# zyang1580/PDA

Measured on AMD Instinct MI355X. Metric: users/sec full-catalogue top-K@50 (eval), higher is better.
Workload: dtype f32; 1 GPU; C3: synthetic 1000000 users x 200000 items, d=128, PDA condition ((elu+1)*pop^0.22) head, masked top-K@50; ranks_seen=1

## Files before the change

pda_amd/csrc/pda_score_topk_v4.hip:

```cpp
#include "pda_v4_shared.h"
#include <cstdlib>
#include <type_traits>

using namespace pda_topk;

namespace {

constexpr int kCap4 = 57;
constexpr int kRing4 = 128;
constexpr int kWarmTiles = 4;
constexpr int kMainWaves = 8;
#ifndef PDA_W4_ABL
#define PDA_W4_ABL 0
#endif
#ifdef PDA_V4_PROF
__device__ unsigned long long pda_prof4[24];
#define PROF_T0(v) const long long v = __builtin_readcyclecounter()
#define PROF_T1(v, slot) prof[slot] += (unsigned long long)(__builtin_readcyclecounter() - v)
#define PROF_INC(slot, x) prof[slot] += (unsigned long long)(x)
#define PROF_FLUSH(first, last) do { if (lane == 0) for (int pq = (first); pq <= (last); ++pq) atomicAdd(&pda_prof4[pq], prof[pq]); } while (0)
#else
#define PROF_T0(v) do {} while (0)
#define PROF_T1(v, slot) do {} while (0)
#define PROF_INC(slot, x) do {} while (0)
// ... 565 lines not shown
        const int row = (r & 3) + 8 * (r >> 2) + 4 * h;
        const int lrow = wave * 32 + row;
        if (j == 0) predt[lrow] = c_t >= K ? pda_unordf(t) : -INFINITY;
        if (__any(c_t > cap_t)) {
#pragma unroll
            for (int k = 0; k < NHT; ++k) {
                const bool p = ordv[k][r] >= t;
                const uint64_t key = ((uint64_t)ordv[k][r] << 32) | (uint64_t)(0xFFFFFFFFu - (uint32_t)itemv[k]);
                append_keys<CAP>(p, lrow, pda_unordf(ordv[k][r]), key, lists, cntl, taul, wave * 32, 32, K, lane);
            }
        } else {
            int run = 0;
#pragma unroll
            for (int k = 0; k < NHT; ++k) {
                const bool p = ordv[k][r] >= t;
                const uint64_t bm = __ballot(p);
                const uint32_t bh = h ? (uint32_t)(bm >> 32) : (uint32_t)bm;
                const int slot = run + __popc(bh & ((1u << j) - 1u));
                if (p) lists[(size_t)lrow * CAP + slot] = ((uint64_t)ordv[k][r] << 32) | (uint64_t)(0xFFFFFFFFu - (uint32_t)itemv[k]);
                run += __popc(bh);
            }
            if (j == 0) cntl[lrow] = run;
        }
    };
#pragma unroll
    for (int r = 0; r < 16; r += 2) {
        if constexpr ((PDA_W4_ABL & 2) != 0) {
#if defined(__HIP_DEVICE_COMPILE__)
#pragma unroll
            for (int k = 0; k < NHT; ++k) asm volatile("" ::"v"(ordv[k][r]), "v"(ordv[k][r + 1]));
#endif
            continue;
        }
        auto count_ge2 = [&](uint32_t ca, uint32_t cb, int& na, int& nb) __attribute__((always_inline)) {
            int loa = 0, hia = 0, lob = 0, hib = 0;
#pragma unroll
            for (int k = 0; k < NHT; ++k) {
                const uint64_t bma = __ballot(ordv[k][r] >= ca);
                const uint64_t bmb = __ballot(ordv[k][r + 1] >= cb);
                loa += __popc((uint32_t)bma);
                hia += __popc((uint32_t)(bma >> 32));
                lob += __popc((uint32_t)bmb);
                hib += __popc((uint32_t)(bmb >> 32));
            }
            na = h ? hia : loa;
            nb = h ? hib : lob;
        };
        int ca_t, cb_t;
        count_ge2(1u, 1u, ca_t, cb_t);
        uint32_t ta = 1u, tb = 1u;
        const bool needa = ca_t > cap_t, needb = cb_t > cap_t;
        if (__any(needa || needb)) {
            uint32_t mxa = 0u, mna = 0xFFFFFFFFu, mxb = 0u, mnb = 0xFFFFFFFFu;
#pragma unroll
            for (int k = 0; k < NHT; ++k) {
                const uint32_t va = ordv[k][r], vb = ordv[k][r + 1];
                mxa = max(mxa, va);
                mna = min(mna, va != 0u ? va : 0xFFFFFFFFu);
                mxb = max(mxb, vb);
                mnb = min(mnb, vb != 0u ? vb : 0xFFFFFFFFu);
            }
#pragma unroll
            for (int o = 16; o >= 1; o >>= 1) {
                mxa = max(mxa, (uint32_t)__shfl_xor((int)mxa, o, 64));
                mna = min(mna, (uint32_t)__shfl_xor((int)mna, o, 64));
                mxb = max(mxb, (uint32_t)__shfl_xor((int)mxb, o, 64));
                mnb = min(mnb, (uint32_t)__shfl_xor((int)mnb, o, 64));
            }
            uint32_t hia = mxa + 1u, hib = mxb + 1u;
            if (needa) ta = mna;
            if (needb) tb = mnb;
            for (int it = 0; it < 40; ++it) {
                const bool opena = needa && ca_t > cap_t && hia - ta > 1u;
                const bool openb = needb && cb_t > cap_t && hib - tb > 1u;
                if (!__any(opena || openb)) break;
                const uint32_t mida = opena ? ta + ((hia - ta) >> 1) : ta;
                const uint32_t midb = openb ? tb + ((hib - tb) >> 1) : tb;
                int cnta, cntb;
                count_ge2(mida, midb, cnta, cntb);
                if (opena) {
                    if (cnta >= K) {
                        ta = mida;
                        ca_t = cnta;
                    } else {
                        hia = mida;
                    }
                }
                if (openb) {
                    if (cntb >= K) {
                        tb = midb;
                        cb_t = cntb;
                    } else {
                        hib = midb;
                    }
                }
            }
        }
        emit_row(r, ta, ca_t);
        emit_row(r + 1, tb, cb_t);
    }
    pda_wave_sync();
    if (tid == 0) atomicAdd(reinterpret_cast<unsigned long long*>(g.stats + 2), (unsigned long long)(2 * nwarm));
    for (int rr = 0; rr < 32; ++rr) {
        uint64_t* buf = my_lists + rr * CAP;
        if (((PDA_W4_ABL & 4) == 0) && (g.warm_sorted || g.warm_final || (g.handover == nullptr && __builtin_amdgcn_readfirstlane(cntl[wave * 32 + rr]) > K)))
            compact_list<CAP>(buf, &cntl[wave * 32 + rr], &taul[wave * 32 + rr], K, lane);
        const int c = cntl[wave * 32 + rr];
        const int rb = utile * kUserTile + wave * 32 + rr;
        if (g.seed_out != nullptr) {
            uint32_t mn = lane < c ? (uint32_t)(buf[lane] >> 32) : 0xFFFFFFFFu;
#pragma unroll
            for (int o = 32; o >= 1; o >>= 1) mn = min(mn, (uint32_t)__shfl_xor((int)mn, o, 64));
            if (lane == 0 && rb < g.n_users_blk) g.seed_out[rb] = c >= K ? pda_unordf(mn) : -INFINITY;
        }
        if (g.kth_ws != nullptr) continue;
        if (g.handover != nullptr) {
            if (rb < g.n_users_blk && lane < CAP) g.handover[((size_t)split * g.n_users_blk + rb) * CAP + lane] = lane < c ? buf[lane] : 0ull;
            if (g.warm_final && rb < g.n_users_blk && lane < K) g.out_keys[((size_t)split * g.n_users_blk + rb) * K + lane] = lane < c ? buf[lane] : 0ull;
        } else if (rb < g.n_users_blk && lane < K) {
            const uint64_t k = lane < c ? buf[lane] : 0ull;
            g.out_keys[((size_t)split * g.n_users_blk + rb) * K + lane] = k;
        }
    }
    if (g.kth_ws != nullptr) {
        pda_wave_sync();
        const int rb0 = utile * kUserTile + wave * 32, nv = max(0, min(32, g.n_users_blk - rb0));
        if (lane < nv) {
            const uint64_t kl = my_lists[(size_t)lane * CAP + (K - 1)];
            g.kth_ws[(size_t)split * g.n_users_blk + rb0 + lane] = cntl[wave * 32 + lane] >= K ? pda_unordf((uint32_t)(kl >> 32)) : -INFINITY;
        }
        uint64_t* ob = g.out_keys + ((size_t)split * g.n_users_blk + rb0) * K;
        const int q64 = 64 / K, r64 = 64 % K;
        int rr = lane / K, p = lane % K;
        for (int i = lane; i < nv * K; i += 64) {
            ob[i] = p < cntl[wave * 32 + rr] ? my_lists[(size_t)rr * CAP + p] : 0ull;
            rr += q64;
            p += r64;
            if (p >= K) { p -= K; ++rr; }
        }
    }
    if (g.pred_ws != nullptr && lane < 32) {
        const int rb = utile * kUserTile + wave * 32 + lane;
        if (rb < g.n_users_blk) {
            g.pred_ws[2 * (size_t)rb] = predt[wave * 32 + lane];
            g.pred_ws[2 * (size_t)rb + 1] = nul[wave * 32 + lane];
        }
    }
}

constexpr int kWS5Waves = 8, kWS5Threads = 64 * kWS5Waves;
constexpr int kWarmPos = 64 * kWarmTiles;
constexpr size_t warm_score5_lds(int d) { return (size_t)kWarmPos * d * 4 + kWarmPos * 8 + (size_t)kWS5Waves * 32 * 2 * kWarmTiles * 4; }

template <int D, bool BF>
__global__ void __launch_bounds__(kWS5Threads) warm_score5_kernel(Args4 g) {
    extern __shared__ __attribute__((aligned(16))) unsigned char smem[];
    constexpr int RB = row_bytes(D);
    constexpr int NC = D / 8;
    constexpr int CPR4 = D / 4;
    float* Bt = reinterpret_cast<float*>(smem);
    float* popw = Bt + kWarmPos * D;
    int* idw = reinterpret_cast<int*>(popw + kWarmPos);
    unsigned* hmask = reinterpret_cast<unsigned*>(idw + kWarmPos);

    const int tid = threadIdx.x, lane = tid & 63, wave = tid >> 6;
    const int j = lane & 31, h = lane >> 5;
    const int nwarm = g.warm_tiles;
    const int npos = 64 * nwarm;
    for (int p = tid; p < npos; p += kWS5Threads) {
        const float* tl = reinterpret_cast<const float*>(g.rows + (size_t)p * RB + 2 * D + 32);
        popw[p] = tl[0];
        idw[p] = reinterpret_cast<const int*>(tl)[1];
    }
    __syncthreads();
    for (int id = tid; id < npos * CPR4; id += kWS5Threads) {
        const int jj = id / CPR4, ch = id % CPR4;
        *reinterpret_cast<f32x4*>(Bt + jj * D + 4 * (ch ^ swz<D>(jj & 31))) = pda_load4<BF>(g.I, (size_t)idw[jj] * D + 4 * ch);
    }
    if (blockIdx.x == 0) {
        for (int p = tid; p < kWarmPos; p += kWS5Threads) g.wscore[p] = p < npos ? (uint32_t)idw[p] : 0u;
        if (tid == 0) g.stats[8] = 5u;
    }
    __syncthreads();

    uint32_t* scores = g.wscore + kWarmPos;
    const int utiles_w = (g.n_users_blk + kUserTile - 1) / kUserTile;
    const int nunits = utiles_w * (kUserTile / 32);
    const int G = (int)gridDim.x, stride = G * kWS5Waves;
    unsigned* hm_l = hmask + wave * 32 * 2 * kWarmTiles;
    static_assert(2 * kWarmTiles == 8, "two 16-byte loads per row");

    auto row_uid = [&](int unit) -> int {
        const int rb = unit * 32 + j;
        return (unit < nunits && rb < g.n_users_blk) ? g.users[rb] : 0;
    };
    auto load_rows = [&](int unit_x, int uid, f32x4 (&a)[NC], u32x4& hm, bool& hm_on) __attribute__((always_inline)) {
        if (unit_x >= nunits) return;
        const int rb = unit_x * 32 + j;
#pragma unroll
        for (int c = 0; c < NC; ++c) a[c] = pda_load4<BF>(g.U, (size_t)uid * D + 4 * h + 8 * c);
        hm_on = false;
        if (g.hmask_tab != nullptr) {
            hm_on = rb < g.n_users_blk && (unsigned)uid < (unsigned)g.hmask_tab_rows;
            hm = *reinterpret_cast<const u32x4*>(g.hmask_tab + (size_t)(hm_on ? uid : 0) * (2 * kWarmTiles) + 4 * h);
        } else if (g.hmask_ws != nullptr) {
            hm_on = true;
            hm = *reinterpret_cast<const u32x4*>(g.hmask_ws + (size_t)rb * (2 * kWarmTiles) + 4 * h);
        }
    };
    unsigned long long n_tiles_done = 0ull;
    auto run_unit = [&](const int unit_in, f32x4 (&areg)[NC], const u32x4& hm_in, const bool hm_on) __attribute__((always_inline)) {
        const int unit = __builtin_amdgcn_readfirstlane(unit_in);
        const int row_blk = unit * 32 + j;
        if (unit * 32 + 32 > g.n_users_blk) {
            const f32x4 z = {0.f, 0.f, 0.f, 0.f};
#pragma unroll
            for (int c = 0; c < NC; ++c) areg[c] = row_blk < g.n_users_blk ? areg[c] : z;
        }
        const u32x4 hz = {0u, 0u, 0u, 0u};
        const u32x4 hmv = hm_on ? hm_in : hz;
        *reinterpret_cast<u32x4*>(hm_l + j * (2 * kWarmTiles) + 4 * h) = hmv;
        {
            constexpr int NK5 = D / 32;
            unsigned char* fb = g.ufrag_out + ((size_t)(row_blk >> 4) * (NK5 * 64) + (size_t)(row_blk & 15)) * 16 + 8 * h;
            float ssc[NC];
#pragma unroll
            for (int c = 0; c < NC; ++c) {
                const f32x4 v = areg[c];
                uint2 w;
                w.x = bf16_rne(v[0]) | (bf16_rne(v[1]) << 16);
                w.y = bf16_rne(v[2]) | (bf16_rne(v[3]) << 16);
                *reinterpret_cast<uint2*>(fb + ((c >> 2) * 64 + 16 * (c & 3)) * 16) = w;
                float ss = 0.f;
#pragma unroll
                for (int k = 0; k < 4; ++k) {
                    const float sq = v[k] * v[k];
                    ss += sq + __shfl_xor(sq, 32, 64);
                }
                ssc[c] = ss;
                __builtin_amdgcn_sched_barrier(0);
            }
#pragma unroll
            for (int o = NC / 2; o > 0; o >>= 1)
#pragma unroll
                for (int c = 0; c < o; ++c) ssc[c] += ssc[c + o];
            if (h == 0) g.unorm_out[row_blk] = sqrtf(ssc[0]) * 1.0009765625f * 1.0001f;
        }
        if ((unit & (kUserTile / 32 - 1)) == 0) n_tiles_done += (unsigned long long)(2 * nwarm);
        pda_wave_sync();
        const int j_lane = j, h_lane = h;
#pragma unroll 1
        for (int ht = 0; ht < 2 * nwarm; ++ht) {
            int j = j_lane, h = h_lane;
#if defined(__HIP_DEVICE_COMPILE__)
            asm volatile("" : "+v"(j), "+v"(h));
#endif
            const int bswz = swz<D>(j);
            const float* brow = Bt + (ht * 32 + j) * D;
            f32x16 acc0 = zero16v(), acc1 = zero16v();
            f32x4 b0 = *reinterpret_cast<const f32x4*>(brow + 4 * (h ^ bswz));
            f32x4 b1 = *reinterpret_cast<const f32x4*>(brow + 4 * ((2 + h) ^ bswz));
#pragma unroll
            for (int c = 0; c < NC; c += 2) {
                f32x4 n0 = b0, n1 = b1;
                if (c + 2 < NC) {
                    n0 = *reinterpret_cast<const f32x4*>(brow + 4 * ((2 * c + 4 + h) ^ bswz));
                    n1 = *reinterpret_cast<const f32x4*>(brow + 4 * ((2 * c + 6 + h) ^ bswz));
                }
#pragma unroll
                for (int q = 0; q < 4; ++q) {
                    acc0 = __builtin_amdgcn_mfma_f32_32x32x2f32(areg[c][q], b0[q], acc0, 0, 0, 0);
                    acc1 = __builtin_amdgcn_mfma_f32_32x32x2f32(areg[c + 1][q], b1[q], acc1, 0, 0, 0);
                }
                __builtin_amdgcn_sched_barrier(0);
                b0 = n0;
                b1 = n1;
            }
            const f32x16 accx = acc0 + acc1;
            const bool okw = (ht * 32 + j) < g.n_items_local;
            const float pv = popw[ht * 32 + j];
            const unsigned hb_mine = hm_l[j * (2 * kWarmTiles) + ht];
            const bool any_hb = __any(hb_mine != 0u);
            const uint32_t soff = (uint32_t)(unit * 32 + 4 * h) * (uint32_t)npos + (uint32_t)(ht * 32 + j);
#pragma unroll
            for (int r = 0; r < 16; ++r) {
                const int row = (r & 3) + 8 * (r >> 2) + 4 * h;
                float sc = accx[r];
                sc = (sc > 0.0f ? sc + 1.0f : __expf(sc)) * pv;
                bool p = okw && (sc >= -INFINITY);
                if (any_hb) {
                    const uint32_t hbr = (uint32_t)__shfl((int)hb_mine, row, 64);
                    if ((hbr >> j) & 1u) p = false;
                }
                scores[soff + (uint32_t)((r & 3) + 8 * (r >> 2)) * (uint32_t)npos] = p ? pda_ordf(sc + 0.0f) : 0u;
            }
        }
        pda_wave_sync();
    };
    int unit = (int)blockIdx.x + G * wave;
    f32x4 ra[NC], rb_[NC];
    u32x4 ha = {0u, 0u, 0u, 0u}, hb = {0u, 0u, 0u, 0u};
    bool oa = false, ob = false;
    load_rows(unit, row_uid(unit), ra, ha, oa);
    int uid_n = row_uid(unit + stride);
    while (unit < nunits) {
        load_rows(unit + stride, uid_n, rb_, hb, ob);
        uid_n = row_uid(unit + 2 * stride);
        run_unit(unit, ra, ha, oa);
        unit += stride;
        if (unit >= nunits) break;
        load_rows(unit + stride, uid_n, ra, ha, oa);
        uid_n = row_uid(unit + 2 * stride);
        run_unit(unit, rb_, hb, ob);
        unit += stride;
    }
    if (lane == 0 && n_tiles_done != 0ull) atomicAdd(reinterpret_cast<unsigned long long*>(g.stats + 2), n_tiles_done);
    if ((int)blockIdx.x == (nunits - 1) % G) {
        const size_t r0 = (size_t)utiles_w * kUserTile, r1 = ((size_t)g.n_users_blk + kUT5 - 1) / kUT5 * kUT5;
        const u32x4 z = {0u, 0u, 0u, 0u};
        for (size_t q = r0 * (2 * D) + (size_t)tid * 16; q < r1 * (2 * D); q += (size_t)kWS5Threads * 16) *reinterpret_cast<u32x4*>(g.ufrag_out + q) = z;
        for (size_t r = r0 + tid; r < r1; r += kWS5Threads) g.unorm_out[r] = 0.f;
    }
}

constexpr int kSelRows = 16;
__global__ void __launch_bounds__(256) __attribute__((amdgpu_waves_per_eu(8))) warm_select5_kernel(Args4 g) {
    constexpr int CAP = kCap4;
    __shared__ uint64_t lists[4][2][64];
    const int tid = threadIdx.x, lane = tid & 63, wave = tid >> 6;
    const int K = g.K, n = g.n_users_blk;
    const int npos = 64 * g.warm_tiles;
    const uint32_t* scores = g.wscore + kWarmPos;
    const int rb0 = ((int)blockIdx.x * 4 + wave) * kSelRows;
    if (rb0 >= n) return;
    const u32x4 idv = *reinterpret_cast<const u32x4*>(g.wscore + 4 * lane);
    uint32_t klo[4];
#pragma unroll
    for (int q = 0; q < 4; ++q) klo[q] = 0xFFFFFFFFu - (uint32_t)(g.item_offset + (int)idv[q]);
    const bool lane_on = 4 * lane < npos;
    float kth_mine = -INFINITY;

    auto count32 = [&](const u32x4& v, uint32_t t) __attribute__((always_inline)) -> int {
        return __popcll(__ballot(v[0] >= t)) + __popcll(__ballot(v[1] >= t)) + __popcll(__ballot(v[2] >= t)) + __popcll(__ballot(v[3] >= t));
    };
    auto key_of = [&](const u32x4& v, int q) __attribute__((always_inline)) -> uint64_t { return ((uint64_t)v[q] << 32) | (uint64_t)klo[q]; };
    auto count64 = [&](const u32x4& v, uint64_t t) __attribute__((always_inline)) -> int {
        int c = 0;
#pragma unroll
        for (int q = 0; q < 4; ++q) c += __popcll(__ballot(key_of(v, q) >= t));
        return c;
    };

#pragma unroll 1
    for (int it = 0; it < kSelRows; it += 2) {
        if (rb0 + it >= n) break;
        u32x4 v[2];
        uint32_t t[2], hi[2];
        int ct[2];
        bool need[2];
#pragma unroll
        for (int s = 0; s < 2; ++s) {
            const int rb = rb0 + it + s;
            const u32x4 z = {0u, 0u, 0u, 0u};
            v[s] = (lane_on && rb < n) ? *reinterpret_cast<const u32x4*>(scores + (size_t)rb * npos + 4 * lane) : z;
        }
#pragma unroll
        for (int s = 0; s < 2; ++s) {
            ct[s] = count32(v[s], 1u);
            t[s] = 1u;
            hi[s] = 0u;
            need[s] = ct[s] > CAP;
        }
        if (need[0] || need[1]) {
#pragma unroll
            for (int s = 0; s < 2; ++s) {
                uint32_t mx = max(max(v[s][0], v[s][1]), max(v[s][2], v[s][3])), mn = 0xFFFFFFFFu;
#pragma unroll
                for (int q = 0; q < 4; ++q) mn = min(mn, v[s][q] != 0u ? v[s][q] : 0xFFFFFFFFu);
#pragma unroll
                for (int o = 32; o >= 1; o >>= 1) {
                    mx = max(mx, (uint32_t)__shfl_xor((int)mx, o, 64));
                    mn = min(mn, (uint32_t)__shfl_xor((int)mn, o, 64));
                }
                hi[s] = (uint32_t)__builtin_amdgcn_readfirstlane((int)mx) + 1u;
                if (need[s]) t[s] = (uint32_t)__builtin_amdgcn_readfirstlane((int)mn);
            }
            for (int step = 0; step < 40; ++step) {
                const bool open0 = need[0] && ct[0] > CAP && hi[0] - t[0] > 1u;
                const bool open1 = need[1] && ct[1] > CAP && hi[1] - t[1] > 1u;
                if (!(open0 || open1)) break;
                const uint32_t mid0 = open0 ? t[0] + ((hi[0] - t[0]) >> 1) : t[0];
                const uint32_t mid1 = open1 ? t[1] + ((hi[1] - t[1]) >> 1) : t[1];
                const int c0 = count32(v[0], mid0), c1 = count32(v[1], mid1);
                if (open0) {
                    if (c0 >= K) { t[0] = mid0; ct[0] = c0; } else { hi[0] = mid0; }
                }
                if (open1) {
                    if (c1 >= K) { t[1] = mid1; ct[1] = c1; } else { hi[1] = mid1; }
                }
            }
        }
        uint64_t thr[2];
#pragma unroll
        for (int s = 0; s < 2; ++s) {
            thr[s] = (uint64_t)t[s] << 32;
            if (ct[s] > CAP) {
                uint64_t lo64 = thr[s], hi64 = (uint64_t)(t[s] + 1u) << 32;
                for (int step = 0; step < 40 && ct[s] > CAP && hi64 - lo64 > 1ull; ++step) {
                    const uint64_t mid = lo64 + ((hi64 - lo64) >> 1);
                    const int c = count64(v[s], mid);
                    if (c >= K) { lo64 = mid; ct[s] = c; } else { hi64 = mid; }
                }
                thr[s] = lo64;
            }
        }
        int cs[2];
#pragma unroll
        for (int s = 0; s < 2; ++s) {
            uint64_t* buf = lists[wave][s];
            int run = 0;
#pragma unroll
            for (int q = 0; q < 4; ++q) {
                const uint64_t key = key_of(v[s], q);
                const bool p = key >= thr[s];
                const uint64_t bm = __ballot(p);
                const int slot = run + (int)__builtin_amdgcn_mbcnt_hi((uint32_t)(bm >> 32), __builtin_amdgcn_mbcnt_lo((uint32_t)bm, 0));
                if (p && slot < 64) buf[slot] = key;
                run += __popcll(bm);
            }
            cs[s] = min(run, CAP);
            if (lane >= cs[s]) buf[lane] = 0ull;
        }
        pda_wave_sync();
        uint64_t key[2];
        int rank[2] = {0, 0};
        key[0] = lists[wave][0][lane];
        key[1] = lists[wave][1][lane];
        const int cm = max(cs[0], cs[1]);
        for (int jj = 0; jj < cm; jj += 4) {
#pragma unroll
            for (int s = 0; s < 2; ++s) {
                const uint64_t* buf = lists[wave][s];
                const uint64_t k0 = buf[jj], k1 = buf[jj + 1], k2 = buf[jj + 2], k3 = buf[jj + 3];
                rank[s] += ((k0 > key[s]) ? 1 : 0) + ((k1 > key[s]) ? 1 : 0) + ((k2 > key[s]) ? 1 : 0) + ((k3 > key[s]) ? 1 : 0);
            }
        }
        pda_wave_sync();
#pragma unroll
        for (int s = 0; s < 2; ++s)
            if (lane < cs[s]) lists[wave][s][rank[s]] = key[s];
        pda_wave_sync();
#pragma unroll
        for (int s = 0; s < 2; ++s) {
            const int rb = rb0 + it + s;
            if (rb < n) {
                if (lane < K) g.out_keys[(size_t)rb * K + lane] = lists[wave][s][lane];
                const uint64_t kl = lists[wave][s][K - 1];
                if (lane == it + s) kth_mine = cs[s] >= K ? pda_unordf((uint32_t)(kl >> 32)) : -INFINITY;
            }
        }
        pda_wave_sync();
    }
    if (lane < kSelRows && rb0 + lane < n) {
        g.kth_ws[rb0 + lane] = kth_mine;
        if (g.seed_out != nullptr) g.seed_out[rb0 + lane] = kth_mine;
    }
}


// ... 1172 lines not shown
    if (mask_from_table) {
        g.hmask_tab = mask_table;
        g.hmask_tab_rows = mask_table_rows;
    }
    if (c.mask_kernel) g.hmask_ws = reinterpret_cast<uint32_t*>(wsb + W.hmask);
    if (c.regroup) {
        g.regroup_ws = reinterpret_cast<int32_t*>(wsb + W.regroup);
        if (phase & 1) g.pred_ws = reinterpret_cast<float*>(g.regroup_ws + 1024 + 2 * (size_t)n_users_blk);
    }

    if (counters_reset && hipMemsetAsync(workspace, 0, W.lists, s) != hipSuccess) return PDA_ERR_LAUNCH;
    if (c.bloom) {
        hipLaunchKernelGGL(hist_bloom4_kernel, dim3((unsigned)((n_users_blk + 31) / 32)), dim3(256), 0, s, users, hist_indptr, hist_indices,
                           hist_row_mode, n_users_blk, const_cast<uint32_t*>(g.bloom), g.prep_hdr, pop_head ? 1 : 0);
        PDA_CHECK_LAUNCH();
    }
#define PDA_V4_(DD, BFV) (pop_head ? launch4<DD, PDA_HEAD_POP, BFV>(g, c, s) : launch4<DD, PDA_HEAD_RAW, BFV>(g, c, s))
    switch (d) {
        case 64: return bf16 ? PDA_V4_(64, true) : PDA_V4_(64, false);
        case 128: return bf16 ? PDA_V4_(128, true) : PDA_V4_(128, false);
        case 256: return bf16 ? PDA_V4_(256, true) : PDA_V4_(256, false);
        default: return PDA_ERR_UNSUPPORTED;
    }
#undef PDA_V4_
}

__global__ void __launch_bounds__(256) kth_value_kernel(const uint64_t* __restrict__ keys, int S, int n_users, int K, int pos, float* __restrict__ out) {
    const int u = blockIdx.x * 256 + threadIdx.x;
    if (u >= n_users) return;
    float best = -INFINITY;
    for (int sp = 0; sp < S; ++sp) {
        const uint64_t k = keys[((size_t)sp * n_users + u) * K + pos];
        if (k != 0ull) best = fmaxf(best, pda_key_val(k));
    }
    out[u] = best;
}

__global__ void __launch_bounds__(256) seed_refine_kernel(const uint64_t* __restrict__ keys, int S, int n_users, int K, float* __restrict__ lo,
                                                          float* __restrict__ hi, float* __restrict__ mid, int32_t* __restrict__ counts, int mode) {
    const int u = blockIdx.x * 256 + threadIdx.x;
    if (u >= n_users) return;
    float l = lo[u], h = hi[u];
    if (mode >= 1) {
        if (counts[u] >= K) l = mid[u];
        else h = mid[u];
        lo[u] = l;
        hi[u] = h;
    }
    if (mode <= 1) {
        const bool open = l > -INFINITY && h < INFINITY && h > l;
        const float m = open ? l + 0.5f * (h - l) : l;
        int c = 0;
        for (int sp = 0; sp < S; ++sp) {
            const uint64_t* row = keys + ((size_t)sp * n_users + u) * K;
            for (int q = 0; q < K; ++q) {
                const uint64_t k = row[q];
                if (k == 0ull || pda_key_val(k) < m) break;
                ++c;
            }
        }
        mid[u] = m;
        counts[u] = c;
    }
}


__global__ void __launch_bounds__(256) seed_bounds_kernel(const uint64_t* __restrict__ keys, int S, int n_users, int K, int m,
                                                          float* __restrict__ out) {
    const int u = blockIdx.x * 256 + threadIdx.x;
    if (u >= n_users) return;
    float a = -INFINITY, b = -INFINITY;
    for (int sp = 0; sp < S; ++sp) {
        const uint64_t* row = keys + ((size_t)sp * n_users + u) * K;
        const uint64_t ka = row[K - 1], kb = row[m - 1];
        if (ka != 0ull) a = fmaxf(a, pda_key_val(ka));
        if (kb != 0ull) b = fmaxf(b, pda_key_val(kb));
    }
    out[u] = a;
    out[(size_t)n_users + u] = b;
    out[2 * (size_t)n_users + u] = -b;
}
__device__ __forceinline__ float seed_thr(float lo, float hi, int j, int n_thr) {
    const bool open = lo > -INFINITY && hi < INFINITY && hi > lo;
    return open ? lo + (hi - lo) * ((float)(j + 1) / (float)(n_thr + 1)) : lo;
}
constexpr int kSeedThrMax = 15;
__global__ void __launch_bounds__(256) seed_counts_kernel(const uint64_t* __restrict__ keys, int S, int n_users, int K,
                                                          const float* __restrict__ bounds, int n_thr, int32_t* __restrict__ counts) {
    const int u = blockIdx.x * 256 + threadIdx.x;
    if (u >= n_users) return;
    const float lo = fmaxf(bounds[u], -bounds[2 * (size_t)n_users + u]), hi = bounds[(size_t)n_users + u];
    float thr[kSeedThrMax];
    int c[kSeedThrMax];
#pragma unroll
    for (int j = 0; j < kSeedThrMax; ++j) { thr[j] = seed_thr(lo, hi, j < n_thr ? j : 0, n_thr); c[j] = 0; }
    for (int sp = 0; sp < S; ++sp) {
        const uint64_t* row = keys + ((size_t)sp * n_users + u) * K;
        for (int q = 0; q < K; ++q) {
            const uint64_t k = row[q];
            if (k == 0ull) break;
            const float v = pda_key_val(k);
            if (v < thr[0]) break;
#pragma unroll
            for (int j = 0; j < kSeedThrMax; ++j) c[j] += (v >= thr[j]) ? 1 : 0;
        }
    }
#pragma unroll
    for (int j = 0; j < kSeedThrMax; ++j)
        if (j < n_thr) counts[(size_t)j * n_users + u] = c[j];
}
__global__ void __launch_bounds__(256) seed_pick_kernel(const float* __restrict__ bounds, const int32_t* __restrict__ counts, int n_thr,
                                                        int n_users, int K, float* __restrict__ seed) {
    const int u = blockIdx.x * 256 + threadIdx.x;
    if (u >= n_users) return;
    const float lo = fmaxf(bounds[u], -bounds[2 * (size_t)n_users + u]), hi = bounds[(size_t)n_users + u];
    float s = lo;
    for (int j = 0; j < n_thr; ++j)
        if (counts[(size_t)j * n_users + u] >= K) s = fmaxf(s, seed_thr(lo, hi, j, n_thr));
    seed[u] = s;
}

}

int pda_v4_run_score4_dev(const void* U, const void* I_shard, bool bf16, const void* prep, const float* pop_shard, const int32_t* users, int n_users_blk,
                          const int* n_users_dev, int item_offset, int n_items_local, int d, const int64_t* hist_indptr, const int32_t* hist_indices,
                          int hist_row_mode, int K, int head, int early_stop, int n_splits, const float* seed, uint64_t* out_keys, void* workspace, hipStream_t s) {
    return run_score4(U, I_shard, bf16, prep, pop_shard, users, n_users_blk, item_offset, n_items_local, d, hist_indptr, hist_indices, hist_row_mode, K, head,
                      early_stop, n_splits, out_keys, workspace, s, seed != nullptr ? 4 : 3, seed, 0, n_users_dev);
}

extern "C" int pda_topk_seed_bounds(const uint64_t* keys, int n_splits, int n_users_blk, int K, int m, float* bounds, void* stream) {
    if (!keys || !bounds || n_splits < 1 || n_users_blk < 1 || K < 1 || m < 1 || m > K) return PDA_ERR_ARG;
    hipLaunchKernelGGL(seed_bounds_kernel, dim3((unsigned)((n_users_blk + 255) / 256)), dim3(256), 0, reinterpret_cast<hipStream_t>(stream), keys,
                       n_splits, n_users_blk, K, m, bounds);
    PDA_CHECK_LAUNCH();
    return PDA_OK;
}
extern "C" int pda_topk_seed_counts(const uint64_t* keys, int n_splits, int n_users_blk, int K, const float* bounds, int n_thr, int32_t* counts,
                                    void* stream) {
    if (!keys || !bounds || !counts || n_splits < 1 || n_users_blk < 1 || K < 1 || n_thr < 1 || n_thr > kSeedThrMax) return PDA_ERR_ARG;
    hipLaunchKernelGGL(seed_counts_kernel, dim3((unsigned)((n_users_blk + 255) / 256)), dim3(256), 0, reinterpret_cast<hipStream_t>(stream), keys,
                       n_splits, n_users_blk, K, bounds, n_thr, counts);
    PDA_CHECK_LAUNCH();
    return PDA_OK;
}
extern "C" int pda_topk_seed_pick(const float* bounds, const int32_t* counts, int n_thr, int n_users_blk, int K, float* seed, void* stream) {
    if (!bounds || !seed || n_users_blk < 1 || K < 1 || n_thr < 0 || n_thr > kSeedThrMax || (n_thr > 0 && !counts)) return PDA_ERR_ARG;
    hipLaunchKernelGGL(seed_pick_kernel, dim3((unsigned)((n_users_blk + 255) / 256)), dim3(256), 0, reinterpret_cast<hipStream_t>(stream), bounds,
                       counts, n_thr, n_users_blk, K, seed);
    PDA_CHECK_LAUNCH();
    return PDA_OK;
}

#ifdef PDA_V5_EXITPROF
extern "C" int pda_debug_v5_exitprof(unsigned long long* out, int n_workgroups) {
    if (!out || n_workgroups < 1 || n_workgroups > kXpMaxWg) return PDA_ERR_ARG;
    if (hipMemcpyFromSymbol(out, HIP_SYMBOL(pda_v5_exitprof), (size_t)n_workgroups * 4 * kXpWords * sizeof(unsigned long long)) != hipSuccess) return PDA_ERR_LAUNCH;
    return PDA_OK;
}
extern "C" int pda_debug_v5_exitprof_words(void) { return kXpWords; }
extern "C" int pda_debug_v5_tail_pieces(int n) {
    if (n < 0) return PDA_ERR_ARG;
    if (hipMemcpyToSymbol(HIP_SYMBOL(pda_v5_tail_pieces), &n, sizeof(int)) != hipSuccess) return PDA_ERR_LAUNCH;
    return PDA_OK;
}
#endif
#ifdef PDA_V4_PROF
extern "C" int pda_debug_prof4(unsigned long long* out16, int reset) {
    if (hipMemcpyFromSymbol(out16, HIP_SYMBOL(pda_prof4), sizeof(unsigned long long) * 24) != hipSuccess) return PDA_ERR_LAUNCH;
    if (reset) { unsigned long long z[24] = {0}; if (hipMemcpyToSymbol(HIP_SYMBOL(pda_prof4), z, sizeof(z)) != hipSuccess) return PDA_ERR_LAUNCH; }
    return PDA_OK;
}
#endif

extern "C" int pda_score_topk4_auto_splits(int n_users_blk, int n_items_local, int d) {
    if (n_users_blk <= 0 || n_items_local <= 0) return 1;
    const int ut = user_tile4(d);
    const int utiles = (n_users_blk + ut - 1) / ut;
    const int n_tiles = (n_items_local + 63) / 64;
    int s = 1;
    while (utiles * s * 2 <= 256 && s < 64 && n_tiles / (s * 2) >= 3 * kWarmTiles) s *= 2;
    return s;
}

extern "C" size_t pda_item_prep4_bytes(int n_items_local, int d) { return n_items_local > 0 ? prep4_layout(n_items_local, d).total : 0; }

extern "C" int pda_item_prep4_f32(const float* I_shard, const float* pop_shard, const int32_t* order, int n_items_local, int d, void* prep,
                                  void* stream) {
    if (!I_shard || !prep || n_items_local <= 0) return PDA_ERR_ARG;
    return run_prep4(I_shard, false, pop_shard, order, n_items_local, d, prep, reinterpret_cast<hipStream_t>(stream));
}
extern "C" int pda_item_prep4_bf16(const uint16_t* I_shard, const float* pop_shard, const int32_t* order, int n_items_local, int d, void* prep,
                                   void* stream) {
    if (!I_shard || !prep || n_items_local <= 0) return PDA_ERR_ARG;
    return run_prep4(I_shard, true, pop_shard, order, n_items_local, d, prep, reinterpret_cast<hipStream_t>(stream));
}
extern "C" int pda_item_prep7_f32(const float* I_shard, const int32_t* order, int n_items_local, int d, void* prep, void* stream) {
    if (!I_shard || !prep || !order || n_items_local <= 0) return PDA_ERR_ARG;
    return run_prep4(I_shard, false, nullptr, order, n_items_local, d, prep, reinterpret_cast<hipStream_t>(stream), 1);
}
extern "C" int pda_item_prep7_bf16(const uint16_t* I_shard, const int32_t* order, int n_items_local, int d, void* prep, void* stream) {
    if (!I_shard || !prep || !order || n_items_local <= 0) return PDA_ERR_ARG;
    return run_prep4(I_shard, true, nullptr, order, n_items_local, d, prep, reinterpret_cast<hipStream_t>(stream), 1);
}
extern "C" int pda_item_prep4_check(const void* prep, int n_items_local, int d, void* stream) {
    if (!prep || n_items_local <= 0) return PDA_ERR_ARG;
    int bad = 0;
    hipStream_t s = reinterpret_cast<hipStream_t>(stream);
    if (hipMemcpyAsync(&bad, prep, 4, hipMemcpyDeviceToHost, s) != hipSuccess) return PDA_ERR_LAUNCH;
    if (hipStreamSynchronize(s) != hipSuccess) return PDA_ERR_LAUNCH;
    return bad ? PDA_ERR_ARG : PDA_OK;
}

extern "C" int pda_topk_kth_value(const uint64_t* keys, int n_splits, int n_users_blk, int K, int pos, float* out, void* stream) {
    if (!keys || !out || n_splits < 1 || n_users_blk < 1 || K < 1 || pos < 0 || pos >= K) return PDA_ERR_ARG;
    hipLaunchKernelGGL(kth_value_kernel, dim3((unsigned)((n_users_blk + 255) / 256)), dim3(256), 0, reinterpret_cast<hipStream_t>(stream), keys,
                       n_splits, n_users_blk, K, pos, out);
    PDA_CHECK_LAUNCH();
    return PDA_OK;
}

extern "C" int pda_topk_seed_refine(const uint64_t* keys, int n_splits, int n_users_blk, int K, float* lo, float* hi, float* mid,
                                    int32_t* counts, int mode, void* stream) {
    if (!keys || !lo || !hi || !mid || !counts || n_splits < 1 || n_users_blk < 1 || K < 1 || mode < 0 || mode > 2) return PDA_ERR_ARG;
    hipLaunchKernelGGL(seed_refine_kernel, dim3((unsigned)((n_users_blk + 255) / 256)), dim3(256), 0, reinterpret_cast<hipStream_t>(stream), keys,
                       n_splits, n_users_blk, K, lo, hi, mid, counts, mode);
    PDA_CHECK_LAUNCH();
    return PDA_OK;
}

extern "C" int pda_score_topk4_phase_f32(const float* U, const float* I_shard, const void* prep, const float* pop_shard, const int32_t* users,
                                         int n_users_blk, int item_offset, int n_items_local, int d, const int64_t* hist_indptr,
                                         const int32_t* hist_indices, int hist_row_mode, int K, int head, int early_stop, int n_splits,
                                         int phase, int warm_tiles, const float* seed, uint64_t* out_keys, void* workspace, void* stream) {
    if (phase != 1 && phase != 2 && phase != 4) return PDA_ERR_ARG;
    return run_score4(U, I_shard, false, prep, pop_shard, users, n_users_blk, item_offset, n_items_local, d, hist_indptr, hist_indices,
                      hist_row_mode, K, head, early_stop, n_splits, out_keys, workspace, reinterpret_cast<hipStream_t>(stream), phase, seed, warm_tiles);
}
extern "C" int pda_score_topk4_phase_bf16(const uint16_t* U, const uint16_t* I_shard, const void* prep, const float* pop_shard,
                                          const int32_t* users, int n_users_blk, int item_offset, int n_items_local, int d,
                                          const int64_t* hist_indptr, const int32_t* hist_indices, int hist_row_mode, int K, int head,
                                          int early_stop, int n_splits, int phase, int warm_tiles, const float* seed, uint64_t* out_keys,
                                          void* workspace, void* stream) {
    if (phase != 1 && phase != 2 && phase != 4) return PDA_ERR_ARG;
    return run_score4(U, I_shard, true, prep, pop_shard, users, n_users_blk, item_offset, n_items_local, d, hist_indptr, hist_indices,
                      hist_row_mode, K, head, early_stop, n_splits, out_keys, workspace, reinterpret_cast<hipStream_t>(stream), phase, seed, warm_tiles);
}

extern "C" int pda_score_topk4_f32(const float* U, const float* I_shard, const void* prep, const float* pop_shard, const int32_t* users,
                                   int n_users_blk, int item_offset, int n_items_local, int d, const int64_t* hist_indptr,
                                   const int32_t* hist_indices, int hist_row_mode, int K, int head, int early_stop, int n_splits,
                                   uint64_t* out_keys, void* workspace, void* stream) {
    return run_score4(U, I_shard, false, prep, pop_shard, users, n_users_blk, item_offset, n_items_local, d, hist_indptr, hist_indices,
                      hist_row_mode, K, head, early_stop, n_splits, out_keys, workspace, reinterpret_cast<hipStream_t>(stream));
}
extern "C" int pda_score_topk4_bf16(const uint16_t* U, const uint16_t* I_shard, const void* prep, const float* pop_shard, const int32_t* users,
                                    int n_users_blk, int item_offset, int n_items_local, int d, const int64_t* hist_indptr,
                                    const int32_t* hist_indices, int hist_row_mode, int K, int head, int early_stop, int n_splits,
                                    uint64_t* out_keys, void* workspace, void* stream) {
    return run_score4(U, I_shard, true, prep, pop_shard, users, n_users_blk, item_offset, n_items_local, d, hist_indptr, hist_indices,
                      hist_row_mode, K, head, early_stop, n_splits, out_keys, workspace, reinterpret_cast<hipStream_t>(stream));
}

extern "C" int pda_score_topk4_phase_masked_f32(const float* U, const float* I_shard, const void* prep, const float* pop_shard, const int32_t* users,
                                                int n_users_blk, int item_offset, int n_items_local, int d, const int64_t* hist_indptr,
                                                const int32_t* hist_indices, int hist_row_mode, int K, int head, int early_stop, int n_splits,
                                                const uint32_t* mask_table, int mask_table_rows, uint64_t* out_keys, void* workspace, void* stream) {
    if (mask_table != nullptr && mask_table_rows <= 0) return PDA_ERR_ARG;
    return run_score4(U, I_shard, false, prep, pop_shard, users, n_users_blk, item_offset, n_items_local, d, hist_indptr, hist_indices,
                      hist_row_mode, K, head, early_stop, n_splits, out_keys, workspace, reinterpret_cast<hipStream_t>(stream), 3, nullptr, 0, nullptr,
                      mask_table, mask_table_rows);
}
extern "C" int pda_score_topk4_phase_masked_bf16(const uint16_t* U, const uint16_t* I_shard, const void* prep, const float* pop_shard, const int32_t* users,
                                                 int n_users_blk, int item_offset, int n_items_local, int d, const int64_t* hist_indptr,
                                                 const int32_t* hist_indices, int hist_row_mode, int K, int head, int early_stop, int n_splits,
                                                 const uint32_t* mask_table, int mask_table_rows, uint64_t* out_keys, void* workspace, void* stream) {
    if (mask_table != nullptr && mask_table_rows <= 0) return PDA_ERR_ARG;
    return run_score4(U, I_shard, true, prep, pop_shard, users, n_users_blk, item_offset, n_items_local, d, hist_indptr, hist_indices,
                      hist_row_mode, K, head, early_stop, n_splits, out_keys, workspace, reinterpret_cast<hipStream_t>(stream), 3, nullptr, 0, nullptr,
                      mask_table, mask_table_rows);
}

static Args4 mask_args4(const void* prep, const int32_t* users, int n_rows, int item_offset, int n_items_local, int d, const int64_t* hist_indptr,
                        const int32_t* hist_indices, int hist_row_mode, int warm_tiles) {
    const Prep4Layout L = prep4_layout(n_items_local, d);
    const unsigned char* pb = reinterpret_cast<const unsigned char*>(prep);
    Args4 g{};
    g.users = users;
    g.hist_indptr = hist_indptr;
    g.hist_indices = hist_indices;
    g.pos_of = reinterpret_cast<const int*>(pb + L.pos_of);
    g.n_users_blk = n_rows;
    g.item_offset = item_offset;
    g.n_items_local = n_items_local;
    g.hist_row_mode = hist_row_mode;
    g.n_splits = 1;
    g.n_tiles = L.n_tiles;
    g.warm_tiles = warm_tiles;
    return g;
}
extern "C" int pda_score_topk4_phase_mask_table(const void* prep, int n_items_local, int d, int item_offset, const int64_t* hist_indptr,
                                                const int32_t* hist_indices, int n_rows, uint32_t* table, void* stream) {
    if (!prep || !hist_indptr || !hist_indices || !table || n_rows <= 0 || n_items_local <= 0 || item_offset < 0) return PDA_ERR_ARG;
    if (d != 64 && d != 128 && d != 256) return PDA_ERR_UNSUPPORTED;
    const Args4 g = mask_args4(prep, nullptr, n_rows, item_offset, n_items_local, d, hist_indptr, hist_indices, PDA_HIST_BY_BLOCK_ROW, kWarmTiles);
    hipLaunchKernelGGL(warm_mask_table4_kernel, dim3((unsigned)((n_rows + kUserTile - 1) / kUserTile)), dim3(kThreads), 0, reinterpret_cast<hipStream_t>(stream), g, table);
// ... 51 lines not shown
```

Baseline: 34.69 million users/s.

## Restructure warm-score epilogue: transposed hmask, prefetched B chunks, buffer stores

```diff
diff --git a/pda_amd/csrc/pda_score_topk_v4.hip b/pda_amd/csrc/pda_score_topk_v4.hip
--- a/pda_amd/csrc/pda_score_topk_v4.hip
+++ b/pda_amd/csrc/pda_score_topk_v4.hip
@@ -741,6 +741,14 @@
 constexpr int kWarmPos = 64 * kWarmTiles;
 constexpr size_t warm_score5_lds(int d) { return (size_t)kWarmPos * d * 4 + kWarmPos * 8 + (size_t)kWS5Waves * 32 * 2 * kWarmTiles * 4; }
 
+#ifdef PDA_WS5_PROF
+constexpr int kWpMaxWg = 1024, kWpWords = 8;
+__device__ unsigned long long pda_ws5_prof[kWpMaxWg * kWS5Waves * kWpWords];
+#define WP(...) __VA_ARGS__
+#else
+#define WP(...)
+#endif
+
 template <int D, bool BF>
 __global__ void __launch_bounds__(kWS5Threads) warm_score5_kernel(Args4 g) {
     extern __shared__ __attribute__((aligned(16))) unsigned char smem[];
@@ -754,6 +762,7 @@
 
     const int tid = threadIdx.x, lane = tid & 63, wave = tid >> 6;
     const int j = lane & 31, h = lane >> 5;
+    WP(unsigned long long wp[kWpWords] = {0, 0, 0, 0, 0, 0, 0, 0}; const unsigned long long wp_k0 = __builtin_amdgcn_s_memtime();)
     const int nwarm = g.warm_tiles;
     const int npos = 64 * nwarm;
     for (int p = tid; p < npos; p += kWS5Threads) {
@@ -778,6 +787,7 @@
     const int G = (int)gridDim.x, stride = G * kWS5Waves;
     unsigned* hm_l = hmask + wave * 32 * 2 * kWarmTiles;
     static_assert(2 * kWarmTiles == 8, "two 16-byte loads per row");
+    const uint32_t voff = 4u * ((uint32_t)(4 * h) * (uint32_t)npos + (uint32_t)j);
 
     auto row_uid = [&](int unit) -> int {
         const int rb = unit * 32 + j;
@@ -808,7 +818,13 @@
         }
         const u32x4 hz = {0u, 0u, 0u, 0u};
         const u32x4 hmv = hm_on ? hm_in : hz;
-        *reinterpret_cast<u32x4*>(hm_l + j * (2 * kWarmTiles) + 4 * h) = hmv;
+        unsigned any_ht = 0u;
+#pragma unroll
+        for (int q = 0; q < 4; ++q) {
+            hm_l[(4 * h + q) * 32 + j] = hmv[q];
+            const unsigned long long bl = __ballot(hmv[q] != 0u);
+            any_ht |= ((uint32_t)bl != 0u ? 1u << q : 0u) | ((uint32_t)(bl >> 32) != 0u ? 16u << q : 0u);
+        }
         {
             constexpr int NK5 = D / 32;
             unsigned char* fb = g.ufrag_out + ((size_t)(row_blk >> 4) * (NK5 * 64) + (size_t)(row_blk & 15)) * 16 + 8 * h;
@@ -824,7 +840,8 @@
 #pragma unroll
                 for (int k = 0; k < 4; ++k) {
                     const float sq = v[k] * v[k];
-                    ss += sq + __shfl_xor(sq, 32, 64);
+                    const auto sw = __builtin_amdgcn_permlane32_swap(__float_as_uint(sq), __float_as_uint(sq), false, false);
+                    ss += __uint_as_float(sw[0]) + __uint_as_float(sw[1]);
                 }
                 ssc[c] = ss;
                 __builtin_amdgcn_sched_barrier(0);
@@ -838,23 +855,43 @@
         if ((unit & (kUserTile / 32 - 1)) == 0) n_tiles_done += (unsigned long long)(2 * nwarm);
         pda_wave_sync();
         const int j_lane = j, h_lane = h;
+        const __amdgpu_buffer_rsrc_t sres = __builtin_amdgcn_make_buffer_rsrc(scores + (size_t)unit * 32 * (size_t)npos, 0, 32 * npos * 4, 0x00020000);
+        auto first_chunks = [&](int ht, int j, int h, f32x4& b0, f32x4& b1) __attribute__((always_inline)) {
+            const int bswz = swz<D>(j);
+            const float* brow = Bt + (ht * 32 + j) * D;
+            b0 = *reinterpret_cast<const f32x4*>(brow + 4 * (h ^ bswz));
+            b1 = *reinterpret_cast<const f32x4*>(brow + 4 * ((2 + h) ^ bswz));
+        };
+        f32x4 b0, b1;
+        first_chunks(0, j_lane, h_lane, b0, b1);
 #pragma unroll 1
         for (int ht = 0; ht < 2 * nwarm; ++ht) {
             int j = j_lane, h = h_lane;
 #if defined(__HIP_DEVICE_COMPILE__)
             asm volatile("" : "+v"(j), "+v"(h));
 #endif
+            WP(const unsigned long long wp_t0 = __builtin_amdgcn_s_memtime();)
             const int bswz = swz<D>(j);
             const float* brow = Bt + (ht * 32 + j) * D;
             f32x16 acc0 = zero16v(), acc1 = zero16v();
-            f32x4 b0 = *reinterpret_cast<const f32x4*>(brow + 4 * (h ^ bswz));
-            f32x4 b1 = *reinterpret_cast<const f32x4*>(brow + 4 * ((2 + h) ^ bswz));
+            float pv = 0.f;
+            uint32_t mbits = 0u;
 #pragma unroll
             for (int c = 0; c < NC; c += 2) {
                 f32x4 n0 = b0, n1 = b1;
                 if (c + 2 < NC) {
                     n0 = *reinterpret_cast<const f32x4*>(brow + 4 * ((2 * c + 4 + h) ^ bswz));
                     n1 = *reinterpret_cast<const f32x4*>(brow + 4 * ((2 * c + 6 + h) ^ bswz));
+                } else {
+                    pv = popw[ht * 32 + j];
+                    if ((any_ht >> ht) & 1u) {
+#pragma unroll
+                        for (int gq = 0; gq < 4; ++gq) {
+                            const u32x4 mw = *reinterpret_cast<const u32x4*>(hm_l + ht * 32 + 8 * gq + 4 * h);
+#pragma unroll
+                            for (int q = 0; q < 4; ++q) mbits |= ((mw[q] >> j) & 1u) << (4 * gq + q);
+                        }
+                    }
                 }
 #pragma unroll
                 for (int q = 0; q < 4; ++q) {
@@ -865,28 +902,29 @@
                 b0 = n0;
                 b1 = n1;
             }
+            WP(const unsigned long long wp_t1 = __builtin_amdgcn_s_memtime();)
             const f32x16 accx = acc0 + acc1;
+            __builtin_amdgcn_sched_barrier(0);
+            first_chunks(ht + 1 < 2 * nwarm ? ht + 1 : 0, j, h, b0, b1);
+            __builtin_amdgcn_sched_barrier(0);
             const bool okw = (ht * 32 + j) < g.n_items_local;
-            const float pv = popw[ht * 32 + j];
-            const unsigned hb_mine = hm_l[j * (2 * kWarmTiles) + ht];
-            const bool any_hb = __any(hb_mine != 0u);
-            const uint32_t soff = (uint32_t)(unit * 32 + 4 * h) * (uint32_t)npos + (uint32_t)(ht * 32 + j);
+            const uint32_t sht = (uint32_t)ht * 128u;
 #pragma unroll
             for (int r = 0; r < 16; ++r) {
-                const int row = (r & 3) + 8 * (r >> 2) + 4 * h;
                 float sc = accx[r];
                 sc = (sc > 0.0f ? sc + 1.0f : __expf(sc)) * pv;
                 bool p = okw && (sc >= -INFINITY);
-                if (any_hb) {
-                    const uint32_t hbr = (uint32_t)__shfl((int)hb_mine, row, 64);
-                    if ((hbr >> j) & 1u) p = false;
-                }
-                scores[soff + (uint32_t)((r & 3) + 8 * (r >> 2)) * (uint32_t)npos] = p ? pda_ordf(sc + 0.0f) : 0u;
-            }
-        }
+                if ((mbits >> r) & 1u) p = false;
+                __builtin_amdgcn_raw_buffer_store_b32(p ? pda_ordf(sc + 0.0f) : 0u, sres, voff, sht + (uint32_t)((r & 3) + 8 * (r >> 2)) * (uint32_t)(4 * npos), 0);
+            }
+            WP(const unsigned long long wp_t2 = __builtin_amdgcn_s_memtime(); const unsigned long long wp_m = wp_t1 - wp_t0, wp_p = wp_t2 - wp_t1;
+               wp[0] += wp_m; wp[1] += wp_p; wp[3] += 1; wp[6] = wp_m > wp[6] ? wp_m : wp[6]; wp[7] = wp_p > wp[7] ? wp_p : wp[7];)
+        }
+        WP(wp[4] += 1;)
         pda_wave_sync();
     };
     int unit = (int)blockIdx.x + G * wave;
+    WP(const unsigned long long wp_u0 = __builtin_amdgcn_s_memtime();)
     f32x4 ra[NC], rb_[NC];
     u32x4 ha = {0u, 0u, 0u, 0u}, hb = {0u, 0u, 0u, 0u};
     bool oa = false, ob = false;
@@ -904,6 +942,8 @@
         unit += stride;
     }
     if (lane == 0 && n_tiles_done != 0ull) atomicAdd(reinterpret_cast<unsigned long long*>(g.stats + 2), n_tiles_done);
+    WP(const unsigned long long wp_e = __builtin_amdgcn_s_memtime(); wp[2] = wp_e - wp_u0; wp[5] = wp_e - wp_k0;
+       if (lane == 0 && blockIdx.x < (unsigned)kWpMaxWg) for (int q = 0; q < kWpWords; ++q) pda_ws5_prof[((size_t)blockIdx.x * kWS5Waves + wave) * kWpWords + q] = wp[q];)
     if ((int)blockIdx.x == (nunits - 1) % G) {
         const size_t r0 = (size_t)utiles_w * kUserTile, r1 = ((size_t)g.n_users_blk + kUT5 - 1) / kUT5 * kUT5;
         const u32x4 z = {0u, 0u, 0u, 0u};
@@ -2382,6 +2422,14 @@
     return PDA_OK;
 }
 
+#ifdef PDA_WS5_PROF
+extern "C" int pda_debug_ws5_prof(unsigned long long* out, int n_workgroups) {
+    if (out == nullptr || n_workgroups <= 0 || n_workgroups > kWpMaxWg) return PDA_ERR_ARG;
+    if (hipMemcpyFromSymbol(out, HIP_SYMBOL(pda_ws5_prof), (size_t)n_workgroups * kWS5Waves * kWpWords * sizeof(unsigned long long)) != hipSuccess) return PDA_ERR_LAUNCH;
+    return PDA_OK;
+}
+extern "C" int pda_debug_ws5_prof_words(void) { return kWpWords; }
+#endif
 #ifdef PDA_V5_EXITPROF
 extern "C" int pda_debug_v5_exitprof(unsigned long long* out, int n_workgroups) {
     if (!out || n_workgroups < 1 || n_workgroups > kXpMaxWg) return PDA_ERR_ARG;
```

After: 34.73 million users/s, median of 6. Within noise of the previous version (+0.1%).
